# jteutenberg/downpore

Hardware: AMD Instinct MI355X
Metric: overlaps/sec (all-vs-all PAF) (higher is better)
Workload: dtype u64

## Files before the change

### downpore_amd/csrc/dp_kbuild.hip

```cpp
#include <algorithm>
#include <cstdio>
#include <cstdlib>
#include <cstring>

#include "dp_common.h"

typedef unsigned long long kb_u64;

#define KB_TILE 16384
#define KB_THREADS 1024
#define KB_P3_CAP 8192

struct KbGeom {
    int k, b1, b2, r;
    int pbits, rbits;
    uint32_t dlo, dhi;
};

struct KbBuf {
    uint32_t* lo;
    void* hi;
    int hb;
};
__device__ __forceinline__ kb_u64 kb_ld(const KbBuf B, kb_u64 i) {
    if (B.hb == 8) return ((const kb_u64*)B.lo)[i];
    kb_u64 v = B.lo[i];
    if (B.hb == 1) v |= (kb_u64)((const uint8_t*)B.hi)[i] << 32;
    else if (B.hb == 2) v |= (kb_u64)((const uint16_t*)B.hi)[i] << 32;
    else if (B.hb == 4) v |= (kb_u64)((const uint32_t*)B.hi)[i] << 32;
    return v;
}
__device__ __forceinline__ void kb_st(const KbBuf B, kb_u64 i, kb_u64 v) {
    if (B.hb == 8) {
        ((kb_u64*)B.lo)[i] = v;
        return;
    }
    B.lo[i] = (uint32_t)v;
    if (B.hb == 1) ((uint8_t*)B.hi)[i] = (uint8_t)(v >> 32);
    else if (B.hb == 2) ((uint16_t*)B.hi)[i] = (uint16_t)(v >> 32);
    else if (B.hb == 4) ((uint32_t*)B.hi)[i] = (uint32_t)(v >> 32);
}

__global__ void kb_group_table(const uint64_t* __restrict__ boff, uint32_t n_reads, uint32_t* __restrict__ gread) {
    const uint32_t r = blockIdx.x * blockDim.x + threadIdx.x;
    if (r >= n_reads) return;
    const uint64_t a0 = boff[r] * 4, a1 = boff[r + 1] * 4;
    for (uint64_t j = (a0 + 1023) >> 10; (j << 10) < a1; j++) gread[j] = r;
}

__device__ __forceinline__ uint32_t kb_read_of(uint64_t a, const uint32_t* __restrict__ gread, const uint64_t* __restrict__ boff) {
    uint32_t r = gread[a >> 10];
    while (boff[r + 1] * 4 <= a) r++;
    return r;
}

__device__ __forceinline__ uint32_t kb_load16(const uint8_t* __restrict__ packed, const uint64_t* __restrict__ boff,
                                              const uint32_t* __restrict__ len, const uint32_t* __restrict__ gread, uint64_t n_groups,
                                              uint64_t g, int half, int k, uint32_t kmer[16], uint32_t* read_out = nullptr,
                                              uint64_t* start_out = nullptr) {
    if (g >= n_groups) return 0u;
    const uint64_t a = g * 32 + (uint64_t)half * 16;
    const uint32_t r = kb_read_of(g * 32, gread, boff);
    const uint32_t L = len[r];
    if (L < (uint32_t)k) return 0u;
    const uint64_t a0 = boff[r] * 4, a1 = a0 + (L - k + 1);
    if (read_out) *read_out = r;
    if (start_out) *start_out = a0;
    if (a >= a1) return 0u;
    const uint32_t* p = (const uint32_t*)(packed + g * 8) + half;
    const uint32_t w0 = __builtin_bswap32(p[0]), w1 = __builtin_bswap32(p[1]);
    const int sh = 32 - 2 * k;
    uint32_t mask = 0;
#pragma unroll
    for (int j = 0; j < 16; j++) {
        const uint32_t win = j ? __builtin_amdgcn_alignbit(w0, w1, 32 - 2 * j) : w0;
        kmer[j] = win >> sh;
        if (a + j >= a0 && a + j < a1) mask |= 1u << j;
    }
    return mask;
}

__global__ __launch_bounds__(KB_THREADS) void kb_count1(const uint8_t* __restrict__ packed, const uint64_t* __restrict__ boff,
                                                        const uint32_t* __restrict__ len, const uint32_t* __restrict__ gread,
                                                        uint64_t n_groups, KbGeom G, kb_u64* __restrict__ cnt1) {
    __shared__ uint32_t hist[1024];
    const int nb = 1 << G.b1;
    for (int i = threadIdx.x; i < nb; i += KB_THREADS) hist[i] = 0;
    __syncthreads();
    const int dsh = 2 * G.k - G.b1;
    const uint64_t tiles = (n_groups * 2 + KB_THREADS - 1) / KB_THREADS;
    for (uint64_t t = blockIdx.x; t < tiles; t += gridDim.x) {
        const uint64_t h = t * KB_THREADS + threadIdx.x;
        uint32_t kmer[16];
        const uint32_t m = kb_load16(packed, boff, len, gread, n_groups, h >> 1, (int)(h & 1), G.k, kmer);
#pragma unroll
        for (int j = 0; j < 16; j++)
            if ((m >> j) & 1) atomicAdd(&hist[kmer[j] >> dsh], 1u);
    }
    __syncthreads();
    for (int i = threadIdx.x; i < nb; i += KB_THREADS)
        if (hist[i]) atomicAdd(&cnt1[i], (kb_u64)hist[i]);
}

template <int E>
__device__ __forceinline__ void kb_tile_out(const kb_u64 (&e)[E], uint32_t m, int dshift, uint32_t dmask, uint32_t* hist ,
                                            uint32_t* lstart , kb_u64* gbase , kb_u64* sorted ,
                                            kb_u64* __restrict__ cursor, const KbBuf out) {
    const int nb = (int)dmask + 1;
    for (int i = threadIdx.x; i < nb; i += KB_THREADS) hist[i] = 0;
    __syncthreads();
    uint32_t rk[E];
#pragma unroll
    for (int j = 0; j < E; j++) rk[j] = ((m >> j) & 1) ? atomicAdd(&hist[(uint32_t)(e[j] >> dshift) & dmask], 1u) : 0u;
    __syncthreads();
    {
        const int per = (nb + KB_THREADS - 1) / KB_THREADS;
        uint32_t loc[4] = {0, 0, 0, 0}, s = 0;
        for (int u = 0; u < per; u++) {
            const int b = threadIdx.x * per + u;
            loc[u] = b < nb ? hist[b] : 0u;
            s += loc[u];
        }
        const int lane = dp_lane(), wave = threadIdx.x >> 6;
        __shared__ uint32_t wsum[KB_THREADS / 64];
        uint32_t x = (uint32_t)wave_incl_sum((int)s);
        if (lane == 63) wsum[wave] = x;
        __syncthreads();
        uint32_t base = x - s;
        for (int w = 0; w < wave; w++) base += wsum[w];
        for (int u = 0; u < per; u++) {
            const int b = threadIdx.x * per + u;
            if (b < nb) {
                lstart[b] = base;
                if (loc[u]) gbase[b] = atomicAdd(&cursor[b], (kb_u64)loc[u]);
                base += loc[u];
            }
        }
    }
    __syncthreads();
    uint32_t total = 0;
#pragma unroll
    for (int j = 0; j < E; j++)
        if ((m >> j) & 1) {
            const uint32_t d = (uint32_t)(e[j] >> dshift) & dmask;
            sorted[lstart[d] + rk[j]] = e[j];
        }
    __syncthreads();
    total = lstart[nb - 1] + hist[nb - 1];
    for (uint32_t i = threadIdx.x; i < total; i += KB_THREADS) {
        const kb_u64 v = sorted[i];
        const uint32_t d = (uint32_t)(v >> dshift) & dmask;
        kb_st(out, gbase[d] + (kb_u64)(i - lstart[d]), v);
    }
    __syncthreads();
}

__global__ __launch_bounds__(KB_THREADS) void kb_part1(const uint8_t* __restrict__ packed, const uint64_t* __restrict__ boff,
                                                       const uint32_t* __restrict__ len, const uint32_t* __restrict__ gread,
                                                       uint64_t n_groups, KbGeom G, kb_u64* __restrict__ cursor, const KbBuf out) {
    __shared__ uint32_t hist[1024], lstart[1024];
    __shared__ kb_u64 gbase[1024];
    __shared__ kb_u64 sorted[KB_TILE];
    const int pay = G.pbits + G.rbits;
    const int dsh = pay + 2 * G.k - G.b1;
    const uint32_t dmask = (1u << G.b1) - 1u;
    const uint64_t tiles = (n_groups * 2 + KB_THREADS - 1) / KB_THREADS;
    for (uint64_t t = blockIdx.x; t < tiles; t += gridDim.x) {
        const uint64_t h = t * KB_THREADS + threadIdx.x;
        uint32_t kmer[16], rd = 0;
        uint64_t a0 = 0;
        const uint32_t m = kb_load16(packed, boff, len, gread, n_groups, h >> 1, (int)(h & 1), G.k, kmer, &rd, &a0);
        kb_u64 e[16];
        const kb_u64 a = (h >> 1) * 32 + (h & 1) * 16;
        const kb_u64 low = ((kb_u64)rd << G.pbits) + (a - a0);
        uint32_t mine = m;
        const int ksh = 2 * G.k - G.b1;
#pragma unroll
        for (int j = 0; j < 16; j++) {
            e[j] = ((kb_u64)kmer[j] << pay) | (low + (kb_u64)j);
            const uint32_t d = kmer[j] >> ksh;
            if (d < G.dlo || d >= G.dhi) mine &= ~(1u << j);
        }
        kb_tile_out<16>(e, mine, dsh, dmask, hist, lstart, gbase, sorted, cursor, out);
    }
}

__device__ __forceinline__ uint32_t kb_bucket_of_tile(const uint32_t* __restrict__ tile_start, int nb1, uint32_t t) {
    int lo = 0, hi = nb1;
    while (hi - lo > 1) {
        const int mid = (lo + hi) >> 1;
        if (tile_start[mid] <= t) lo = mid;
        else hi = mid;
    }
    return (uint32_t)lo;
}

__global__ __launch_bounds__(KB_THREADS) void kb_count2(const KbBuf in, const kb_u64* __restrict__ base1,
                                                        const uint32_t* __restrict__ tile_start, KbGeom G, kb_u64* __restrict__ cnt2) {
    __shared__ uint32_t hist[1024];
    const int nb1 = 1 << G.b1, nb2 = 1 << G.b2;
    const uint32_t n_tiles = tile_start[nb1];
    const int dsh = G.pbits + G.rbits + 2 * G.k - G.b1 - G.b2;
    const uint32_t dmask = (uint32_t)nb2 - 1u;
    for (uint32_t t = blockIdx.x; t < n_tiles; t += gridDim.x) {
        const uint32_t b = kb_bucket_of_tile(tile_start, nb1, t);
        const kb_u64 lo = base1[b] + (kb_u64)(t - tile_start[b]) * KB_TILE, hi = min(base1[b + 1], lo + KB_TILE);
        for (int i = threadIdx.x; i < nb2; i += KB_THREADS) hist[i] = 0;
        __syncthreads();
        for (kb_u64 i = lo + threadIdx.x; i < hi; i += KB_THREADS) atomicAdd(&hist[(uint32_t)(kb_ld(in, i) >> dsh) & dmask], 1u);
        __syncthreads();
        for (int i = threadIdx.x; i < nb2; i += KB_THREADS)
            if (hist[i]) atomicAdd(&cnt2[(kb_u64)b * nb2 + i], (kb_u64)hist[i]);
        __syncthreads();
    }
}

__global__ __launch_bounds__(KB_THREADS) void kb_part2(const KbBuf in, const kb_u64* __restrict__ base1,
                                                       const uint32_t* __restrict__ tile_start, KbGeom G, kb_u64* __restrict__ cursor2,
                                                       const KbBuf out) {
    __shared__ uint32_t hist[1024], lstart[1024];
    __shared__ kb_u64 gbase[1024];
    __shared__ kb_u64 sorted[KB_TILE];
    const int nb1 = 1 << G.b1, nb2 = 1 << G.b2;
    const uint32_t n_tiles = tile_start[nb1];
    const int dsh = G.pbits + G.rbits + 2 * G.k - G.b1 - G.b2;
    const uint32_t dmask = (uint32_t)nb2 - 1u;
    for (uint32_t t = blockIdx.x; t < n_tiles; t += gridDim.x) {
        const uint32_t b = kb_bucket_of_tile(tile_start, nb1, t);
        const kb_u64 lo = base1[b] + (kb_u64)(t - tile_start[b]) * KB_TILE, hi = min(base1[b + 1], lo + KB_TILE);
        kb_u64 e[KB_TILE / KB_THREADS];
        uint32_t m = 0;
#pragma unroll
        for (int j = 0; j < KB_TILE / KB_THREADS; j++) {
            const kb_u64 i = lo + (kb_u64)j * KB_THREADS + threadIdx.x;
            e[j] = 0;
            if (i < hi) {
                e[j] = kb_ld(in, i);
                m |= 1u << j;
            }
        }
        kb_tile_out<KB_TILE / KB_THREADS>(e, m, dsh, dmask, hist, lstart, gbase, sorted, cursor2 + (kb_u64)b * nb2, out);
    }
}

struct KbPosOut {
    void* lo;
    uint8_t* hi;
    int fmt;
};
__device__ __forceinline__ void kb_pos_st(const KbPosOut P, kb_u64 i, kb_u64 v, const KbGeom& G) {
    const kb_u64 pay = v & (((kb_u64)1 << (G.pbits + G.rbits)) - 1);
    if (P.fmt == 8) {
        ((kb_u64*)P.lo)[i] = ((pay >> G.pbits) << 32) | (pay & (((kb_u64)1 << G.pbits) - 1));
    } else {
        ((uint32_t*)P.lo)[i] = (uint32_t)pay;
        if (P.fmt == 5) P.hi[i] = (uint8_t)(pay >> 32);
    }
}
__global__ __launch_bounds__(KB_THREADS) void kb_final(const KbBuf in, const kb_u64* __restrict__ base2, uint32_t n_sub,
                                                       KbGeom G, const uint32_t* __restrict__ gread, const uint64_t* __restrict__ boff,
                                                       uint32_t* __restrict__ counts, kb_u64* __restrict__ off, const KbPosOut pos) {
    extern __shared__ kb_u64 kb_dyn[];
    const int nb = 1 << G.r;
    kb_u64* sorted = kb_dyn;
    uint32_t* hist = (uint32_t*)(kb_dyn + KB_P3_CAP);
    uint32_t* lstart = hist + nb;
    const uint32_t dmask = (uint32_t)nb - 1u;
    const int pay = G.pbits + G.rbits;
    for (uint32_t sp = blockIdx.x; sp < n_sub; sp += gridDim.x) {
        const kb_u64 lo = base2[sp], hi = base2[sp + 1];
        const kb_u64 n = hi - lo;
        for (int i = threadIdx.x; i < nb; i += KB_THREADS) hist[i] = 0;
        __syncthreads();
        constexpr int KB_HOLD = KB_P3_CAP / KB_THREADS;
        kb_u64 held[KB_HOLD];
        uint32_t rk[KB_HOLD];
        const bool hold = n <= KB_P3_CAP;
        if (hold) {
#pragma unroll
            for (int u = 0; u < KB_HOLD; u++) {
                const kb_u64 i = lo + (kb_u64)u * KB_THREADS + threadIdx.x;
                held[u] = i < hi ? kb_ld(in, i) : 0;
                rk[u] = i < hi ? atomicAdd(&hist[(uint32_t)(held[u] >> pay) & dmask], 1u) : 0u;
            }
        } else {
            for (kb_u64 i = lo + threadIdx.x; i < hi; i += KB_THREADS) atomicAdd(&hist[(uint32_t)(kb_ld(in, i) >> pay) & dmask], 1u);
        }
        __syncthreads();
        {
            const int per = (nb + KB_THREADS - 1) / KB_THREADS;
            uint32_t s = 0;
            for (int u = 0; u < per; u++) {
                const int b = threadIdx.x * per + u;
                if (b < nb) s += hist[b];
            }
            const int lane = dp_lane(), wave = threadIdx.x >> 6;
            __shared__ uint32_t wsum[KB_THREADS / 64];
            uint32_t x = (uint32_t)wave_incl_sum((int)s);
            if (lane == 63) wsum[wave] = x;
            __syncthreads();
            uint32_t base = x - s;
            for (int w = 0; w < wave; w++) base += wsum[w];
            for (int u = 0; u < per; u++) {
                const int b = threadIdx.x * per + u;
                if (b < nb) {
                    lstart[b] = base;
                    base += hist[b];
                }
            }
        }
        __syncthreads();
        const kb_u64 kbase = (kb_u64)sp << G.r;
        for (int b = threadIdx.x; b < nb; b += KB_THREADS) {
            counts[kbase + b] = hist[b];
            off[kbase + b] = lo + lstart[b];
        }
        if (hold) {
#pragma unroll
            for (int u = 0; u < KB_HOLD; u++) {
                const kb_u64 i = lo + (kb_u64)u * KB_THREADS + threadIdx.x;
                if (i < hi) {
                    const kb_u64 v = held[u];
                    const uint32_t d = (uint32_t)(v >> pay) & dmask;
                    sorted[lstart[d] + rk[u]] = v;
                }
            }
            __syncthreads();
            for (uint32_t i = threadIdx.x; i < (uint32_t)n; i += KB_THREADS) {
                kb_pos_st(pos, lo + i, sorted[i], G);
            }
        } else {
            __syncthreads();
            for (int i = threadIdx.x; i < nb; i += KB_THREADS) hist[i] = 0;
            __syncthreads();
            for (kb_u64 i = lo + threadIdx.x; i < hi; i += KB_THREADS) {
                const kb_u64 v = kb_ld(in, i);
                const uint32_t d = (uint32_t)(v >> pay) & dmask;
                kb_pos_st(pos, lo + lstart[d] + atomicAdd(&hist[d], 1u), v, G);
            }
        }
        __syncthreads();
    }
    if (blockIdx.x == 0 && threadIdx.x == 0) off[(kb_u64)n_sub << G.r] = base2[n_sub];
}

__global__ void kb_mask_digits(kb_u64* __restrict__ cnt1, uint32_t nb1, uint32_t dlo, uint32_t dhi) {
    const uint32_t d = blockIdx.x * blockDim.x + threadIdx.x;
    if (d < nb1 && (d < dlo || d >= dhi)) cnt1[d] = 0;
}

__global__ void kb_excl_scan_small(const kb_u64* __restrict__ in, uint32_t n, kb_u64* __restrict__ out) {
    __shared__ kb_u64 part[1024];
    const uint32_t per = (((n + 1023) / 1024) + 15u) & ~15u;
    const uint32_t lo = min(n, threadIdx.x * per), hi = min(n, lo + per);
    kb_u64 s = 0;
    for (uint32_t i = lo; i < hi; i += 16) {
        kb_u64 v[16];
#pragma unroll
        for (int j = 0; j < 16; j++) v[j] = i + j < hi ? in[i + j] : 0;
#pragma unroll
        for (int j = 0; j < 16; j++) s += v[j];
    }
    part[threadIdx.x] = s;
    __syncthreads();
    for (int d = 1; d < 1024; d <<= 1) {
        const kb_u64 v = (int)threadIdx.x >= d ? part[threadIdx.x - d] : 0;
        __syncthreads();
        part[threadIdx.x] += v;
        __syncthreads();
    }
    kb_u64 run = part[threadIdx.x] - s;
    for (uint32_t i = lo; i < hi; i += 16) {
        kb_u64 v[16];
#pragma unroll
        for (int j = 0; j < 16; j++) v[j] = i + j < hi ? in[i + j] : 0;
#pragma unroll
        for (int j = 0; j < 16; j++) {
            if (i + j < hi) out[i + j] = run;
            run += v[j];
        }
    }
    if (threadIdx.x == 1023) out[n] = run;
}

__global__ __launch_bounds__(1024) void kb_scan_partials(const kb_u64* __restrict__ in, uint32_t n, uint32_t chunk, kb_u64* __restrict__ partial) {
    __shared__ kb_u64 red[16];
    const uint32_t lo = min(n, blockIdx.x * chunk), hi = min(n, lo + chunk);
    kb_u64 s = 0;
    for (uint32_t i = lo + threadIdx.x; i < hi; i += 1024) s += in[i];
    for (int o = 32; o > 0; o >>= 1) s += __shfl_xor(s, o, 64);
    if (dp_lane() == 0) red[threadIdx.x >> 6] = s;
    __syncthreads();
    if (threadIdx.x == 0) {
        kb_u64 t = 0;
        for (int w = 0; w < 16; w++) t += red[w];
        partial[blockIdx.x] = t;
    }
}
__global__ __launch_bounds__(1024) void kb_scan_write(const kb_u64* __restrict__ in, uint32_t n, uint32_t chunk, const kb_u64* __restrict__ pbase,
                                                      kb_u64* __restrict__ out) {
    __shared__ kb_u64 part[1024];
    const uint32_t lo = min(n, blockIdx.x * chunk), hi = min(n, lo + chunk);
    kb_u64 run = pbase[blockIdx.x];
    for (uint32_t b0 = lo; b0 < hi; b0 += 1024) {
        const uint32_t i = b0 + threadIdx.x;
        const kb_u64 v = i < hi ? in[i] : 0;
        part[threadIdx.x] = v;
        __syncthreads();
        for (int d = 1; d < 1024; d <<= 1) {
            const kb_u64 u = (int)threadIdx.x >= d ? part[threadIdx.x - d] : 0;
            __syncthreads();
            part[threadIdx.x] += u;
            __syncthreads();
        }
        if (i < hi) out[i] = run + part[threadIdx.x] - v;
        run += part[1023];
        __syncthreads();
    }
    if (blockIdx.x == gridDim.x - 1 && threadIdx.x == 0) out[n] = run;
}

int dp_kindex_build_sorted(dp_ctx* ctx, dp_ctx* ow, int k, uint32_t* d_counts, uint64_t* d_off, void** d_pos_out, void** d_pos_hi_out,
                           int* fmt_out, int* pbits_out, uint64_t* n_pos_out, float* ms_out, dp_kindex_shard* shard) {
    if (k < 9 || k > 14 || ow->n_reads == 0) return 1;
    if (dp_tune("kindex_atomic", 0)) return 1;
    const uint64_t n_groups = (ow->packed_bytes * 4 + 31) / 32;
    KbGeom G;
    G.k = k;
    {
        uint32_t max_len = 1;
        for (uint32_t r = 0; r < ow->n_reads; r++) max_len = std::max(max_len, ow->h_len[r]);
        G.pbits = 1;
        while (((uint64_t)1 << G.pbits) <= max_len) G.pbits++;
        G.rbits = 1;
        while (((uint64_t)1 << G.rbits) < ow->n_reads) G.rbits++;
        G.pbits = std::max(G.pbits, (int)dp_env_long("DP_KB_MIN_PBITS", 0, LONG_MIN, 32));
        if (2 * k + G.pbits + G.rbits > 64) return 1;
    }
    const int pay = G.pbits + G.rbits;
    G.b1 = 8;
    G.b1 = (int)std::max(6L, std::min(10L, dp_tune("kb_b1", G.b1)));
    if (G.b1 > 2 * k - 2) G.b1 = 2 * k - 2;
    const uint64_t approx = ow->total_bases;
    int b2 = std::max(1, 14 - G.b1);
    while (b2 < 10 && (approx >> (G.b1 + b2)) > 7800) b2++;
    if (G.b1 + b2 > 2 * k) b2 = 2 * k - G.b1;
    G.b2 = b2;
    G.r = 2 * k - G.b1 - G.b2;
    if (G.r > 12) {
        G.b2 += G.r - 12;
        G.r = 12;
    }
    if (G.b2 > 10) return 1;
    const int nb1 = 1 << G.b1, nb2 = 1 << G.b2;
    G.dlo = 0;
    G.dhi = (uint32_t)nb1;
    const uint32_t n_sub = (uint32_t)nb1 * (uint32_t)nb2;
    const bool wide = dp_env_str("DP_KINDEX_WIDE") != nullptr;
    const int hb1 = 8, hb2 = 8;
    (void)wide;
    const int fmt = (wide || pay > 40) ? 8 : pay > 32 ? 5 : 4;
    const bool a_lo_wide = hb1 == 8 || fmt == 8;
    const bool f_over_a = a_lo_wide == (fmt == 8);
    {
        const uint64_t per_entry = (uint64_t)((a_lo_wide ? 8 : 4) + (hb1 != 8 ? hb1 : 0)) + (uint64_t)(hb2 == 8 ? 8 : 4 + hb2) + (f_over_a ? 0u : 4u) + (fmt == 5 ? 1u : 0u);
        size_t free_b = 0, total_b = 0;
        hipMemGetInfo(&free_b, &total_b);
        free_b += dp_dev_cached_bytes();
        const uint64_t mine = shard && shard->n_ranks > 1 ? ow->total_bases / (uint64_t)shard->n_ranks + (ow->total_bases >> 6) : ow->total_bases;
        if ((uint64_t)free_b < mine * per_entry + ((uint64_t)6 << 30)) return 1;
    }
    void *d_gread = nullptr, *d_small = nullptr, *d_a_lo = nullptr, *d_a_hi = nullptr, *d_b_lo = nullptr, *d_b_hi = nullptr, *d_f_hi = nullptr;
    struct Temps {
        std::vector<void**> v;
        ~Temps() {
            for (void** p : v)
                if (*p) dp_dev_free(*p);
        }
    } temps{{&d_gread, &d_small, &d_a_lo, &d_a_hi, &d_b_lo, &d_b_hi, &d_f_hi}};
    const size_t n_blocks1k = (size_t)((ow->packed_bytes * 4 + 1023) >> 10) + 2;
    DP_HIP(dp_dev_malloc(&d_gread, n_blocks1k * 4));
    const size_t small_u64 = (size_t)nb1 * 3 + 1 + (size_t)n_sub * 3 + 1;
    DP_HIP(dp_dev_malloc(&d_small, small_u64 * 8 + ((size_t)nb1 + 1) * 4 + 64));
    kb_u64* cnt1 = (kb_u64*)d_small;
    kb_u64* base1 = cnt1 + nb1;
    kb_u64* cur1 = base1 + nb1 + 1;
    kb_u64* cnt2 = cur1 + nb1;
    kb_u64* base2 = cnt2 + n_sub;
    kb_u64* cur2 = base2 + n_sub + 1;
    uint32_t* tile_start = (uint32_t*)(cur2 + n_sub);
    DP_HIP(hipMemsetAsync(d_small, 0, small_u64 * 8 + ((size_t)nb1 + 1) * 4, ctx->stream));
    hipEvent_t e0 = ctx->ev[2], e1 = ctx->ev[3];
    DP_HIP(hipEventRecord(e0, ctx->stream));
    hipLaunchKernelGGL(kb_group_table, dim3((ow->n_reads + 255) / 256), dim3(256), 0, ctx->stream, (const uint64_t*)ow->d_boff.p, ow->n_reads,
                       (uint32_t*)d_gread);
    int cus = 256;
    hipDeviceGetAttribute(&cus, hipDeviceAttributeMultiprocessorCount, ctx->device);
    const uint32_t grid = (uint32_t)cus * 8;
    hipLaunchKernelGGL(kb_count1, dim3(grid), dim3(KB_THREADS), 0, ctx->stream, (const uint8_t*)ow->d_packed.p, (const uint64_t*)ow->d_boff.p,
                       (const uint32_t*)ow->d_len.p, (const uint32_t*)d_gread, n_groups, G, cnt1);
    if (shard) {
        std::vector<kb_u64> h_cnt((size_t)nb1);
        DP_HIP(hipMemcpyAsync(h_cnt.data(), cnt1, (size_t)nb1 * 8, hipMemcpyDeviceToHost, ctx->stream));
        DP_HIP(dp_stream_sync(ctx));
        kb_u64 all = 0;
        for (int b = 0; b < nb1; b++) all += h_cnt[(size_t)b];
        const int N = shard->n_ranks;
        shard->digit_first.assign((size_t)N + 1, (uint32_t)nb1);
        shard->entry_first.assign((size_t)N + 1, all);
        std::vector<kb_u64> pre((size_t)nb1 + 1, 0);
        for (int b = 0; b < nb1; b++) pre[(size_t)b + 1] = pre[(size_t)b] + h_cnt[(size_t)b];
        shard->digit_first[0] = 0;
        shard->entry_first[0] = 0;
        for (int q = 1; q < N; q++) {
            const kb_u64 want = (all * (kb_u64)q + (kb_u64)N - 1) / (kb_u64)N;
            int b = (int)shard->digit_first[(size_t)q - 1];
            while (b < nb1 && pre[(size_t)b] < want) b++;
            shard->digit_first[(size_t)q] = (uint32_t)b;
            shard->entry_first[(size_t)q] = pre[(size_t)b];
        }
        shard->digit_first[(size_t)N] = (uint32_t)nb1;
        shard->entry_first[(size_t)N] = all;
        shard->kmer_shift = 2 * k - G.b1;
        shard->total = all;
        G.dlo = shard->digit_first[(size_t)shard->rank];
        G.dhi = shard->digit_first[(size_t)shard->rank + 1];
        hipLaunchKernelGGL(kb_mask_digits, dim3((nb1 + 255) / 256), dim3(256), 0, ctx->stream, cnt1, (uint32_t)nb1, G.dlo, G.dhi);
    }
    hipLaunchKernelGGL(kb_excl_scan_small, dim3(1), dim3(1024), 0, ctx->stream, (const kb_u64*)cnt1, (uint32_t)nb1, base1);
    DP_HIP(hipGetLastError());
    std::vector<kb_u64> h_base1((size_t)nb1 + 1);
    DP_HIP(hipMemcpyAsync(h_base1.data(), base1, ((size_t)nb1 + 1) * 8, hipMemcpyDeviceToHost, ctx->stream));
    DP_HIP(dp_stream_sync(ctx));
    const uint64_t n = h_base1[(size_t)nb1];
    std::vector<uint32_t> h_tiles((size_t)nb1 + 1);
    uint64_t tt = 0;
    for (int b = 0; b < nb1; b++) {
        h_tiles[(size_t)b] = (uint32_t)tt;
        tt += (h_base1[(size_t)b + 1] - h_base1[(size_t)b] + KB_TILE - 1) / KB_TILE;
    }
    h_tiles[(size_t)nb1] = (uint32_t)tt;
    if (tt >= 0xffffffffull) return 1;
    void* d_f_lo = nullptr;
    temps.v.push_back(&d_f_lo);
#define KB_ALLOC(p_, bytes_)                              \
    if (dp_dev_malloc(&(p_), (bytes_)) != hipSuccess) {   \
        (void)hipGetLastError();                          \
        return 1;                                         \
    }
    KB_ALLOC(d_a_lo, n * (size_t)(a_lo_wide ? 8 : 4) + 64)
    if (hb1 && hb1 != 8) KB_ALLOC(d_a_hi, n * (size_t)hb1 + 64)
    KB_ALLOC(d_b_lo, n * (size_t)(hb2 == 8 ? 8 : 4) + 64)
    if (hb2 && hb2 != 8) KB_ALLOC(d_b_hi, n * (size_t)hb2 + 64)
    if (fmt == 5) KB_ALLOC(d_f_hi, n + 64)
    if (!f_over_a) KB_ALLOC(d_f_lo, n * 4 + 64)
#undef KB_ALLOC
    const KbBuf A = {(uint32_t*)d_a_lo, d_a_hi, hb1}, B = {(uint32_t*)d_b_lo, d_b_hi, hb2};
    const KbPosOut F = {f_over_a ? d_a_lo : d_f_lo, (uint8_t*)d_f_hi, fmt};
    DP_HIP(hipMemcpyAsync(tile_start, h_tiles.data(), ((size_t)nb1 + 1) * 4, hipMemcpyHostToDevice, ctx->stream));
    DP_HIP(hipMemcpyAsync(cur1, base1, (size_t)nb1 * 8, hipMemcpyDeviceToDevice, ctx->stream));
    hipLaunchKernelGGL(kb_part1, dim3(grid), dim3(KB_THREADS), 0, ctx->stream, (const uint8_t*)ow->d_packed.p, (const uint64_t*)ow->d_boff.p,
                       (const uint32_t*)ow->d_len.p, (const uint32_t*)d_gread, n_groups, G, cur1, A);
    hipLaunchKernelGGL(kb_count2, dim3(grid), dim3(KB_THREADS), 0, ctx->stream, A, (const kb_u64*)base1, (const uint32_t*)tile_start, G, cnt2);
    if (n_sub >= 8192) {
        const uint32_t n_wg = 256, chunk = (((n_sub + n_wg - 1) / n_wg) + 1023u) & ~1023u;
        hipLaunchKernelGGL(kb_scan_partials, dim3(n_wg), dim3(1024), 0, ctx->stream, (const kb_u64*)cnt2, n_sub, chunk, cur2);
        hipLaunchKernelGGL(kb_excl_scan_small, dim3(1), dim3(1024), 0, ctx->stream, (const kb_u64*)cur2, n_wg, cur2 + n_wg);
        hipLaunchKernelGGL(kb_scan_write, dim3(n_wg), dim3(1024), 0, ctx->stream, (const kb_u64*)cnt2, n_sub, chunk, (const kb_u64*)(cur2 + n_wg), base2);
    } else {
        hipLaunchKernelGGL(kb_excl_scan_small, dim3(1), dim3(1024), 0, ctx->stream, (const kb_u64*)cnt2, n_sub, base2);
    }
    DP_HIP(hipMemcpyAsync(cur2, base2, (size_t)n_sub * 8, hipMemcpyDeviceToDevice, ctx->stream));
    hipLaunchKernelGGL(kb_part2, dim3(grid), dim3(KB_THREADS), 0, ctx->stream, A, (const kb_u64*)base1, (const uint32_t*)tile_start, G, cur2, B);
    hipLaunchKernelGGL(kb_final, dim3(std::min<uint32_t>(n_sub, (uint32_t)cus * 16)), dim3(KB_THREADS),
                       (size_t)KB_P3_CAP * 8 + ((size_t)8 << G.r), ctx->stream, B, (const kb_u64*)base2, n_sub, G, (const uint32_t*)d_gread,
                       (const uint64_t*)ow->d_boff.p, d_counts, (kb_u64*)d_off, F);
    DP_HIP(hipGetLastError());
    DP_HIP(hipEventRecord(e1, ctx->stream));
    DP_HIP(dp_stream_sync(ctx));
    if (ms_out) hipEventElapsedTime(ms_out, e0, e1);
    *d_pos_out = f_over_a ? d_a_lo : d_f_lo;
    (f_over_a ? d_a_lo : d_f_lo) = nullptr;
    *d_pos_hi_out = d_f_hi;
    d_f_hi = nullptr;
    *fmt_out = fmt;
    *pbits_out = G.pbits;
    *n_pos_out = n;
    return DP_OK;
}
```

Measured before the change: 41.21 million.

## Prefetch next tile's input during k-mer index partition and final sort passes

Splits the per-tile bucket sort into a sort phase and a copy phase so that kb_part1 can issue the packed-sequence fetch for the next tile before writing out the current one. kb_final likewise prefetches the next sub-bucket's bounds and held entries while the current bucket is being scattered. The split-hi/lo KbBuf storage paths are removed in favour of plain 64-bit buffers, which were already the only configuration in use. The prefetching raises register pressure and adds a small amount of extra synchronization logic around histogram resets.

```diff
diff --git a/downpore_amd/csrc/dp_kbuild.hip b/downpore_amd/csrc/dp_kbuild.hip
--- a/downpore_amd/csrc/dp_kbuild.hip
+++ b/downpore_amd/csrc/dp_kbuild.hip
@@ -18,28 +18,10 @@
 };
 
 struct KbBuf {
-    uint32_t* lo;
-    void* hi;
-    int hb;
+    kb_u64* p;
 };
-__device__ __forceinline__ kb_u64 kb_ld(const KbBuf B, kb_u64 i) {
-    if (B.hb == 8) return ((const kb_u64*)B.lo)[i];
-    kb_u64 v = B.lo[i];
-    if (B.hb == 1) v |= (kb_u64)((const uint8_t*)B.hi)[i] << 32;
-    else if (B.hb == 2) v |= (kb_u64)((const uint16_t*)B.hi)[i] << 32;
-    else if (B.hb == 4) v |= (kb_u64)((const uint32_t*)B.hi)[i] << 32;
-    return v;
-}
-__device__ __forceinline__ void kb_st(const KbBuf B, kb_u64 i, kb_u64 v) {
-    if (B.hb == 8) {
-        ((kb_u64*)B.lo)[i] = v;
-        return;
-    }
-    B.lo[i] = (uint32_t)v;
-    if (B.hb == 1) ((uint8_t*)B.hi)[i] = (uint8_t)(v >> 32);
-    else if (B.hb == 2) ((uint16_t*)B.hi)[i] = (uint16_t)(v >> 32);
-    else if (B.hb == 4) ((uint32_t*)B.hi)[i] = (uint32_t)(v >> 32);
-}
+__device__ __forceinline__ kb_u64 kb_ld(const KbBuf B, kb_u64 i) { return B.p[i]; }
+__device__ __forceinline__ void kb_st(const KbBuf B, kb_u64 i, kb_u64 v) { B.p[i] = v; }
 
 __global__ void kb_group_table(const uint64_t* __restrict__ boff, uint32_t n_reads, uint32_t* __restrict__ gread) {
     const uint32_t r = blockIdx.x * blockDim.x + threadIdx.x;
@@ -54,30 +36,39 @@
     return r;
 }
 
-__device__ __forceinline__ uint32_t kb_load16(const uint8_t* __restrict__ packed, const uint64_t* __restrict__ boff,
-                                              const uint32_t* __restrict__ len, const uint32_t* __restrict__ gread, uint64_t n_groups,
-                                              uint64_t g, int half, int k, uint32_t kmer[16], uint32_t* read_out = nullptr,
-                                              uint64_t* start_out = nullptr) {
-    if (g >= n_groups) return 0u;
+struct Kb16 {
+    uint32_t w0, w1, mask;
+    uint32_t read;
+    uint64_t start;
+};
+__device__ __forceinline__ Kb16 kb_fetch16(const uint8_t* __restrict__ packed, const uint64_t* __restrict__ boff,
+                                           const uint32_t* __restrict__ len, const uint32_t* __restrict__ gread, uint64_t n_groups,
+                                           uint64_t g, int half, int k) {
+    Kb16 f = {0u, 0u, 0u, 0u, 0};
+    if (g >= n_groups) return f;
     const uint64_t a = g * 32 + (uint64_t)half * 16;
     const uint32_t r = kb_read_of(g * 32, gread, boff);
     const uint32_t L = len[r];
-    if (L < (uint32_t)k) return 0u;
+    if (L < (uint32_t)k) return f;
     const uint64_t a0 = boff[r] * 4, a1 = a0 + (L - k + 1);
-    if (read_out) *read_out = r;
-    if (start_out) *start_out = a0;
-    if (a >= a1) return 0u;
+    f.read = r;
+    f.start = a0;
+    if (a >= a1) return f;
     const uint32_t* p = (const uint32_t*)(packed + g * 8) + half;
-    const uint32_t w0 = __builtin_bswap32(p[0]), w1 = __builtin_bswap32(p[1]);
+    f.w0 = __builtin_bswap32(p[0]);
+    f.w1 = __builtin_bswap32(p[1]);
+#pragma unroll
+    for (int j = 0; j < 16; j++)
+        if (a + j >= a0 && a + j < a1) f.mask |= 1u << j;
+    return f;
+}
+__device__ __forceinline__ void kb_kmers16(const Kb16& f, int k, uint32_t kmer[16]) {
     const int sh = 32 - 2 * k;
-    uint32_t mask = 0;
 #pragma unroll
     for (int j = 0; j < 16; j++) {
-        const uint32_t win = j ? __builtin_amdgcn_alignbit(w0, w1, 32 - 2 * j) : w0;
+        const uint32_t win = j ? __builtin_amdgcn_alignbit(f.w0, f.w1, 32 - 2 * j) : f.w0;
         kmer[j] = win >> sh;
-        if (a + j >= a0 && a + j < a1) mask |= 1u << j;
-    }
-    return mask;
+    }
 }
 
 __global__ __launch_bounds__(KB_THREADS) void kb_count1(const uint8_t* __restrict__ packed, const uint64_t* __restrict__ boff,
@@ -92,10 +83,11 @@
     for (uint64_t t = blockIdx.x; t < tiles; t += gridDim.x) {
         const uint64_t h = t * KB_THREADS + threadIdx.x;
         uint32_t kmer[16];
-        const uint32_t m = kb_load16(packed, boff, len, gread, n_groups, h >> 1, (int)(h & 1), G.k, kmer);
+        const Kb16 f = kb_fetch16(packed, boff, len, gread, n_groups, h >> 1, (int)(h & 1), G.k);
+        kb_kmers16(f, G.k, kmer);
 #pragma unroll
         for (int j = 0; j < 16; j++)
-            if ((m >> j) & 1) atomicAdd(&hist[kmer[j] >> dsh], 1u);
+            if ((f.mask >> j) & 1) atomicAdd(&hist[kmer[j] >> dsh], 1u);
     }
     __syncthreads();
     for (int i = threadIdx.x; i < nb; i += KB_THREADS)
@@ -103,9 +95,9 @@
 }
 
 template <int E>
-__device__ __forceinline__ void kb_tile_out(const kb_u64 (&e)[E], uint32_t m, int dshift, uint32_t dmask, uint32_t* hist ,
-                                            uint32_t* lstart , kb_u64* gbase , kb_u64* sorted ,
-                                            kb_u64* __restrict__ cursor, const KbBuf out) {
+__device__ __forceinline__ void kb_tile_sort(const kb_u64 (&e)[E], uint32_t m, int dshift, uint32_t dmask, uint32_t* hist ,
+                                             uint32_t* lstart , kb_u64* gbase , kb_u64* sorted ,
+                                             kb_u64* __restrict__ cursor) {
     const int nb = (int)dmask + 1;
     for (int i = threadIdx.x; i < nb; i += KB_THREADS) hist[i] = 0;
     __syncthreads();
@@ -113,14 +105,10 @@
 #pragma unroll
     for (int j = 0; j < E; j++) rk[j] = ((m >> j) & 1) ? atomicAdd(&hist[(uint32_t)(e[j] >> dshift) & dmask], 1u) : 0u;
     __syncthreads();
+    kb_u64 reserved = 0;
     {
-        const int per = (nb + KB_THREADS - 1) / KB_THREADS;
-        uint32_t loc[4] = {0, 0, 0, 0}, s = 0;
-        for (int u = 0; u < per; u++) {
-            const int b = threadIdx.x * per + u;
-            loc[u] = b < nb ? hist[b] : 0u;
-            s += loc[u];
-        }
+        const int b = threadIdx.x;
+        const uint32_t s = b < nb ? hist[b] : 0u;
         const int lane = dp_lane(), wave = threadIdx.x >> 6;
         __shared__ uint32_t wsum[KB_THREADS / 64];
         uint32_t x = (uint32_t)wave_incl_sum((int)s);
@@ -128,25 +116,25 @@
         __syncthreads();
         uint32_t base = x - s;
         for (int w = 0; w < wave; w++) base += wsum[w];
-        for (int u = 0; u < per; u++) {
-            const int b = threadIdx.x * per + u;
-            if (b < nb) {
-                lstart[b] = base;
-                if (loc[u]) gbase[b] = atomicAdd(&cursor[b], (kb_u64)loc[u]);
-                base += loc[u];
-            }
-        }
-    }
-    __syncthreads();
-    uint32_t total = 0;
+        if (b < nb) {
+            lstart[b] = base;
+            if (s) reserved = atomicAdd(&cursor[b], (kb_u64)s);
+        }
+    }
+    __syncthreads();
 #pragma unroll
     for (int j = 0; j < E; j++)
         if ((m >> j) & 1) {
             const uint32_t d = (uint32_t)(e[j] >> dshift) & dmask;
             sorted[lstart[d] + rk[j]] = e[j];
         }
-    __syncthreads();
-    total = lstart[nb - 1] + hist[nb - 1];
+    if ((int)threadIdx.x < nb) gbase[threadIdx.x] = reserved;
+}
+__device__ __forceinline__ void kb_tile_copy(int dshift, uint32_t dmask, const uint32_t* hist, const uint32_t* lstart,
+                                             const kb_u64* gbase, const kb_u64* sorted, const KbBuf out) {
+    const int nb = (int)dmask + 1;
+    __syncthreads();
+    const uint32_t total = lstart[nb - 1] + hist[nb - 1];
     for (uint32_t i = threadIdx.x; i < total; i += KB_THREADS) {
         const kb_u64 v = sorted[i];
         const uint32_t d = (uint32_t)(v >> dshift) & dmask;
@@ -165,15 +153,17 @@
     const int dsh = pay + 2 * G.k - G.b1;
     const uint32_t dmask = (1u << G.b1) - 1u;
     const uint64_t tiles = (n_groups * 2 + KB_THREADS - 1) / KB_THREADS;
-    for (uint64_t t = blockIdx.x; t < tiles; t += gridDim.x) {
-        const uint64_t h = t * KB_THREADS + threadIdx.x;
-        uint32_t kmer[16], rd = 0;
-        uint64_t a0 = 0;
-        const uint32_t m = kb_load16(packed, boff, len, gread, n_groups, h >> 1, (int)(h & 1), G.k, kmer, &rd, &a0);
+    uint64_t t = blockIdx.x;
+    if (t >= tiles) return;
+    uint64_t h = t * KB_THREADS + threadIdx.x;
+    Kb16 f = kb_fetch16(packed, boff, len, gread, n_groups, h >> 1, (int)(h & 1), G.k);
+    for (;;) {
+        uint32_t kmer[16];
+        kb_kmers16(f, G.k, kmer);
         kb_u64 e[16];
         const kb_u64 a = (h >> 1) * 32 + (h & 1) * 16;
-        const kb_u64 low = ((kb_u64)rd << G.pbits) + (a - a0);
-        uint32_t mine = m;
+        const kb_u64 low = ((kb_u64)f.read << G.pbits) + (a - f.start);
+        uint32_t mine = f.mask;
         const int ksh = 2 * G.k - G.b1;
 #pragma unroll
         for (int j = 0; j < 16; j++) {
@@ -181,7 +171,13 @@
             const uint32_t d = kmer[j] >> ksh;
             if (d < G.dlo || d >= G.dhi) mine &= ~(1u << j);
         }
-        kb_tile_out<16>(e, mine, dsh, dmask, hist, lstart, gbase, sorted, cursor, out);
+        kb_tile_sort<16>(e, mine, dsh, dmask, hist, lstart, gbase, sorted, cursor);
+        t += gridDim.x;
+        const bool more = t < tiles;
+        h = t * KB_THREADS + threadIdx.x;
+        if (more) f = kb_fetch16(packed, boff, len, gread, n_groups, h >> 1, (int)(h & 1), G.k);
+        kb_tile_copy(dsh, dmask, hist, lstart, gbase, sorted, out);
+        if (!more) break;
     }
 }
 
@@ -239,7 +235,8 @@
                 m |= 1u << j;
             }
         }
-        kb_tile_out<KB_TILE / KB_THREADS>(e, m, dsh, dmask, hist, lstart, gbase, sorted, cursor2 + (kb_u64)b * nb2, out);
+        kb_tile_sort<KB_TILE / KB_THREADS>(e, m, dsh, dmask, hist, lstart, gbase, sorted, cursor2 + (kb_u64)b * nb2);
+        kb_tile_copy(dsh, dmask, hist, lstart, gbase, sorted, out);
     }
 }
 
@@ -267,20 +264,32 @@
     uint32_t* lstart = hist + nb;
     const uint32_t dmask = (uint32_t)nb - 1u;
     const int pay = G.pbits + G.rbits;
-    for (uint32_t sp = blockIdx.x; sp < n_sub; sp += gridDim.x) {
-        const kb_u64 lo = base2[sp], hi = base2[sp + 1];
+    constexpr int KB_HOLD = KB_P3_CAP / KB_THREADS;
+    kb_u64 held[KB_HOLD];
+    bool fetched = false;
+    uint32_t sp = blockIdx.x;
+    kb_u64 lo = 0, hi = 0;
+    if (sp < n_sub) {
+        lo = base2[sp];
+        hi = base2[sp + 1];
+    }
+    for (int i = threadIdx.x; i < nb; i += KB_THREADS) hist[i] = 0;
+    __syncthreads();
+    while (sp < n_sub) {
         const kb_u64 n = hi - lo;
-        for (int i = threadIdx.x; i < nb; i += KB_THREADS) hist[i] = 0;
-        __syncthreads();
-        constexpr int KB_HOLD = KB_P3_CAP / KB_THREADS;
-        kb_u64 held[KB_HOLD];
         uint32_t rk[KB_HOLD];
         const bool hold = n <= KB_P3_CAP;
         if (hold) {
+            if (!fetched) {
+#pragma unroll
+                for (int u = 0; u < KB_HOLD; u++) {
+                    const kb_u64 i = lo + (kb_u64)u * KB_THREADS + threadIdx.x;
+                    held[u] = i < hi ? kb_ld(in, i) : 0;
+                }
+            }
 #pragma unroll
             for (int u = 0; u < KB_HOLD; u++) {
                 const kb_u64 i = lo + (kb_u64)u * KB_THREADS + threadIdx.x;
-                held[u] = i < hi ? kb_ld(in, i) : 0;
                 rk[u] = i < hi ? atomicAdd(&hist[(uint32_t)(held[u] >> pay) & dmask], 1u) : 0u;
             }
         } else {
@@ -315,6 +324,13 @@
             counts[kbase + b] = hist[b];
             off[kbase + b] = lo + lstart[b];
         }
+        const kb_u64 sp_next = (kb_u64)sp + gridDim.x;
+        kb_u64 lo_next = 0, hi_next = 0;
+        if (sp_next < n_sub) {
+            lo_next = base2[sp_next];
+            hi_next = base2[sp_next + 1];
+        }
+        fetched = false;
         if (hold) {
 #pragma unroll
             for (int u = 0; u < KB_HOLD; u++) {
@@ -325,7 +341,16 @@
                     sorted[lstart[d] + rk[u]] = v;
                 }
             }
+            if (sp_next < n_sub && hi_next - lo_next <= KB_P3_CAP) {
+#pragma unroll
+                for (int u = 0; u < KB_HOLD; u++) {
+                    const kb_u64 i = lo_next + (kb_u64)u * KB_THREADS + threadIdx.x;
+                    held[u] = i < hi_next ? kb_ld(in, i) : 0;
+                }
+                fetched = true;
+            }
             __syncthreads();
+            for (int i = threadIdx.x; i < nb; i += KB_THREADS) hist[i] = 0;
             for (uint32_t i = threadIdx.x; i < (uint32_t)n; i += KB_THREADS) {
                 kb_pos_st(pos, lo + i, sorted[i], G);
             }
@@ -338,8 +363,13 @@
                 const uint32_t d = (uint32_t)(v >> pay) & dmask;
                 kb_pos_st(pos, lo + lstart[d] + atomicAdd(&hist[d], 1u), v, G);
             }
-        }
-        __syncthreads();
+            __syncthreads();
+            for (int i = threadIdx.x; i < nb; i += KB_THREADS) hist[i] = 0;
+        }
+        __syncthreads();
+        sp = sp_next < n_sub ? (uint32_t)sp_next : n_sub;
+        lo = lo_next;
+        hi = hi_next;
     }
     if (blockIdx.x == 0 && threadIdx.x == 0) off[(kb_u64)n_sub << G.r] = base2[n_sub];
 }
@@ -457,27 +487,24 @@
     G.dhi = (uint32_t)nb1;
     const uint32_t n_sub = (uint32_t)nb1 * (uint32_t)nb2;
     const bool wide = dp_env_str("DP_KINDEX_WIDE") != nullptr;
-    const int hb1 = 8, hb2 = 8;
-    (void)wide;
     const int fmt = (wide || pay > 40) ? 8 : pay > 32 ? 5 : 4;
-    const bool a_lo_wide = hb1 == 8 || fmt == 8;
-    const bool f_over_a = a_lo_wide == (fmt == 8);
+    const bool f_over_a = fmt == 8;
     {
-        const uint64_t per_entry = (uint64_t)((a_lo_wide ? 8 : 4) + (hb1 != 8 ? hb1 : 0)) + (uint64_t)(hb2 == 8 ? 8 : 4 + hb2) + (f_over_a ? 0u : 4u) + (fmt == 5 ? 1u : 0u);
+        const uint64_t per_entry = 8u + 8u + (f_over_a ? 0u : 4u) + (fmt == 5 ? 1u : 0u);
         size_t free_b = 0, total_b = 0;
         hipMemGetInfo(&free_b, &total_b);
         free_b += dp_dev_cached_bytes();
         const uint64_t mine = shard && shard->n_ranks > 1 ? ow->total_bases / (uint64_t)shard->n_ranks + (ow->total_bases >> 6) : ow->total_bases;
         if ((uint64_t)free_b < mine * per_entry + ((uint64_t)6 << 30)) return 1;
     }
-    void *d_gread = nullptr, *d_small = nullptr, *d_a_lo = nullptr, *d_a_hi = nullptr, *d_b_lo = nullptr, *d_b_hi = nullptr, *d_f_hi = nullptr;
+    void *d_gread = nullptr, *d_small = nullptr, *d_a = nullptr, *d_b = nullptr, *d_f_hi = nullptr;
     struct Temps {
         std::vector<void**> v;
         ~Temps() {
             for (void** p : v)
                 if (*p) dp_dev_free(*p);
         }
-    } temps{{&d_gread, &d_small, &d_a_lo, &d_a_hi, &d_b_lo, &d_b_hi, &d_f_hi}};
+    } temps{{&d_gread, &d_small, &d_a, &d_b, &d_f_hi}};
     const size_t n_blocks1k = (size_t)((ow->packed_bytes * 4 + 1023) >> 10) + 2;
     DP_HIP(dp_dev_malloc(&d_gread, n_blocks1k * 4));
     const size_t small_u64 = (size_t)nb1 * 3 + 1 + (size_t)n_sub * 3 + 1;
@@ -548,15 +575,13 @@
         (void)hipGetLastError();                          \
         return 1;                                         \
     }
-    KB_ALLOC(d_a_lo, n * (size_t)(a_lo_wide ? 8 : 4) + 64)
-    if (hb1 && hb1 != 8) KB_ALLOC(d_a_hi, n * (size_t)hb1 + 64)
-    KB_ALLOC(d_b_lo, n * (size_t)(hb2 == 8 ? 8 : 4) + 64)
-    if (hb2 && hb2 != 8) KB_ALLOC(d_b_hi, n * (size_t)hb2 + 64)
+    KB_ALLOC(d_a, n * 8 + 64)
+    KB_ALLOC(d_b, n * 8 + 64)
     if (fmt == 5) KB_ALLOC(d_f_hi, n + 64)
     if (!f_over_a) KB_ALLOC(d_f_lo, n * 4 + 64)
 #undef KB_ALLOC
-    const KbBuf A = {(uint32_t*)d_a_lo, d_a_hi, hb1}, B = {(uint32_t*)d_b_lo, d_b_hi, hb2};
-    const KbPosOut F = {f_over_a ? d_a_lo : d_f_lo, (uint8_t*)d_f_hi, fmt};
+    const KbBuf A = {(kb_u64*)d_a}, B = {(kb_u64*)d_b};
+    const KbPosOut F = {f_over_a ? d_a : d_f_lo, (uint8_t*)d_f_hi, fmt};
     DP_HIP(hipMemcpyAsync(tile_start, h_tiles.data(), ((size_t)nb1 + 1) * 4, hipMemcpyHostToDevice, ctx->stream));
     DP_HIP(hipMemcpyAsync(cur1, base1, (size_t)nb1 * 8, hipMemcpyDeviceToDevice, ctx->stream));
     hipLaunchKernelGGL(kb_part1, dim3(grid), dim3(KB_THREADS), 0, ctx->stream, (const uint8_t*)ow->d_packed.p, (const uint64_t*)ow->d_boff.p,
@@ -579,8 +604,8 @@
     DP_HIP(hipEventRecord(e1, ctx->stream));
     DP_HIP(dp_stream_sync(ctx));
     if (ms_out) hipEventElapsedTime(ms_out, e0, e1);
-    *d_pos_out = f_over_a ? d_a_lo : d_f_lo;
-    (f_over_a ? d_a_lo : d_f_lo) = nullptr;
+    *d_pos_out = f_over_a ? d_a : d_f_lo;
+    (f_over_a ? d_a : d_f_lo) = nullptr;
     *d_pos_hi_out = d_f_hi;
     d_f_hi = nullptr;
     *fmt_out = fmt;
```

New measurement: 38.20 million. 0.927x the previous value.
